# cvigilv/SimSpread.jl

Hardware: AMD Instinct MI355X
Metric: predicted edges/sec + achieved HBM GB/s, W*R SpMM (higher is better)
Workload: dtype f32

## Files before the change

simspread.jl_amd/csrc/assemble.hip:

```cpp
#include <cstdlib>
#include <cstring>
#include <hip/hip_runtime.h>
#include <rocprim/rocprim.hpp>

#include "graph.hpp"

namespace ss {

static inline int grid_for(int64_t work, int block, int cap = 256 * 16) {
  int64_t g = ceil_div(work, block);
  if (g < 1) g = 1;
  if (g > cap) g = cap;
  return (int)g;
}

__global__ void scan_tail_kernel(const int* in, int* out, int64_t n) { out[n] = out[n - 1] + in[n - 1]; }

static int exclusive_scan_int(const int* in, int* out, int64_t n) {
  hipStream_t st = ctx().stream;
  if (n == 0) {
    SS_HIP(hipMemsetAsync(out, 0, sizeof(int), st));
    return SS_OK;
  }
  size_t bytes = 0;
// ... 1124 lines not shown
    const int64_t r = i - (int64_t)c * rows;
    const int64_t o = (int64_t)off[i] * align;
    const int npad = (off[i + 1] - off[i]) * align;
    if (npad == 0) continue;
    const int lo = ptr[r], hi = ptr[r + 1];
    const int64_t k0 = (int64_t)c * SC, k1 = k0 + SC;
    int a = lo, b = hi;
    while (a < b) { const int m = (a + b) >> 1; if (idx[m] < k0) a = m + 1; else b = m; }
    const int first = a;
    b = hi;
    while (a < b) { const int m = (a + b) >> 1; if (idx[m] < k1) a = m + 1; else b = m; }
    const int n = a - first;
    if (cls_tails && n > 64) {
      const int cls = (int)(r & 3);
      int m = 0;
      for (int x0 = 0; x0 < n; x0 += 64) {
        const int x = x0 + lane;
        m += __popcll(__ballot(x < n && ((idx[first + x] - k0) & 3) == cls));
      }
      const ChunkTail tl = chunk_tail(n, m);
      int seen_c = 0, seen_o = 0;
      for (int x0 = 0; x0 < n; x0 += 64) {
        const int x = x0 + lane;
        const bool valid = x < n;
        const int col = valid ? (int)(idx[first + x] - k0) : 0;
        const T v = valid ? val[first + x] : T(0);
        const unsigned long long mc = __ballot(valid && (col & 3) == cls);
        const int rc = seen_c + __popcll(mc & below);
        const bool in_tail = valid && (col & 3) == cls && rc < tl.real;
        const unsigned long long mo = __ballot(valid && !in_tail);
        const int ro = seen_o + __popcll(mo & below);
        if (in_tail) {
          oidx[o + 64 + rc] = (unsigned short)col;
          oval[o + 64 + rc] = v;
        } else if (valid) {
          if (ro < 64) {
            hcol[wv][ro] = col;
            hval[wv][ro] = v;
          } else {
            oidx[o + 16 + ro] = (unsigned short)col;
            oval[o + 16 + ro] = v;
          }
        }
        seen_c += __popcll(mc);
        seen_o += __popcll(mo);
      }
      for (int x = tl.real + lane; x < tl.len; x += 64) {
        oidx[o + 64 + x] = (unsigned short)SC;
        oval[o + 64 + x] = T(0);
      }
      __builtin_amdgcn_wave_barrier();
      const int hc = hcol[wv][lane];
      const T hv = hval[wv][lane];
      __builtin_amdgcn_wave_barrier();
      const int pos = sched ? chunk_sched_pos(64, hc, lane) : lane;
      oidx[o + pos] = (unsigned short)hc;
      oval[o + pos] = hv;
      for (int x = tl.stored + lane; x < npad; x += 64) {
        oidx[o + x] = (unsigned short)SC;
        oval[o + x] = T(0);
      }
      continue;
    }
    if (sched && n > 32 && n <= 64) {
      const int col = lane < n ? (int)(idx[first + lane] - k0) : -1;
      const int pos = chunk_sched_pos(n, col, lane);
      if (lane < n) {
        oidx[o + pos] = (unsigned short)col;
        oval[o + pos] = val[first + lane];
      }
      for (int x = n + lane; x < npad; x += 64) {
        oidx[o + x] = (unsigned short)SC;
        oval[o + x] = T(0);
      }
      continue;
    }
    for (int x = lane; x < npad; x += 64) {
      oidx[o + x] = x < n ? (unsigned short)(idx[first + x] - k0) : (unsigned short)SC;
      oval[o + x] = x < n ? val[first + x] : T(0);
    }
  }
}

template <class T>
int chunked_build(const DevCsr<T>& in, int SC, int align, DevChunked<T>& out) {
  hipStream_t st = ctx().stream;
  if (SC < 1 || SC > 65535) return fail(SS_EINVAL, "chunk size out of range");
  if (align != 1 && align != 4 && align != 32) return fail(SS_EINVAL, "chunk alignment must be 1, 4 or 32");
  out.rows = in.rows;
  out.cols = in.cols;
  out.nnz = in.nnz;
  out.SC = SC;
  out.align = align;
  out.binary = in.binary;
  out.nchunks = (int)(in.cols > 0 ? ceil_div(in.cols, SC) : 1);
  const int64_t total = in.rows * out.nchunks;
  SS_TRY(out.off.alloc(total + 1));
  if (total == 0) {
    SS_HIP(hipMemsetAsync(out.off.p, 0, sizeof(int), st));
    SS_TRY(out.idx.alloc(64));
    SS_TRY(out.val.alloc(64));
    SS_HIP(hipMemsetAsync(out.idx.p, 0, 64 * sizeof(unsigned short), st));
    SS_HIP(hipMemsetAsync(out.val.p, 0, 64 * sizeof(T), st));
    return SS_OK;
  }
  DevBuf<int> cnt;
  SS_TRY(cnt.alloc(total));
  const int cls_tails = (align == 1 || align == 32) ? 1 : 0;
  DevBuf<int> toolong;
  if (align == 32) {
    SS_TRY(out.len.alloc(total));
    SS_TRY(toolong.alloc(1));
    SS_HIP(hipMemsetAsync(toolong.p, 0, sizeof(int), st));
  }
  hipLaunchKernelGGL(chunk_count_kernel, dim3(grid_for(total, 256)), dim3(256), 0, st, in.ptr.p, in.idx.p, in.rows, SC,
                     out.nchunks, align, cls_tails, cnt.p, align == 32 ? out.len.p : (unsigned short*)nullptr,
                     align == 32 ? toolong.p : (int*)nullptr);
  SS_LAUNCH_CHECK();
  if (align == 32) {
    int tl = 0;
    SS_TRY(read_int(toolong.p, &tl));
    out.len_ok = (tl == 0);
  }
  {
    DevBuf<int> mm;
    SS_TRY(mm.alloc(2));
    const int init[2] = {0, 0x7f7fffff};
    SS_HIP(hipMemcpyAsync(mm.p, init, sizeof(init), hipMemcpyHostToDevice, st));
    if (in.nnz > 0) {
      hipLaunchKernelGGL(abs_range_kernel<T>, dim3(grid_for(in.nnz, 256)), dim3(256), 0, st, in.val.p, in.nnz, mm.p);
      SS_LAUNCH_CHECK();
    }
    int got[2];
    SS_HIP(hipMemcpyAsync(got, mm.p, sizeof(got), hipMemcpyDeviceToHost, st));
    SS_HIP(hipStreamSynchronize(st));
    memcpy(&out.vmax, &got[0], 4);
    memcpy(&out.vmin, &got[1], 4);
    if (in.nnz == 0) out.vmax = out.vmin = 0.f;
  }
  SS_TRY(exclusive_scan_int(cnt.p, out.off.p, total));
  int units = 0;
  SS_TRY(read_int(out.off.p + total, &units));
  if (units < 0 || (int64_t)units * align >= (1LL << 31) - 64) return fail(SS_EUNSUPPORTED, "chunked operand too large");
  out.stored = (int64_t)units * align;
  SS_TRY(out.idx.alloc(out.stored + 256));
  SS_TRY(out.val.alloc(out.stored + 256));
  SS_HIP(hipMemsetAsync(out.idx.p + out.stored, 0, 256 * sizeof(unsigned short), st));
  SS_HIP(hipMemsetAsync(out.val.p + out.stored, 0, 256 * sizeof(T), st));
  const int sched = (cls_tails && !env_off("SS_CHUNK_SCHED")) ? 1 : 0;
  hipLaunchKernelGGL(chunk_fill_kernel<T>, dim3(grid_for(total * 64, 256)), dim3(256), 0, st, in.ptr.p, in.idx.p,
                     in.val.p, in.rows, SC, out.nchunks, align, sched, cls_tails, out.off.p, out.idx.p, out.val.p);
  SS_LAUNCH_CHECK();
  SS_HIP(hipStreamSynchronize(st));
  return SS_OK;
}

template <class T>
__global__ void degree_kernel(const int* __restrict__ pa, const int* __restrict__ pb, int64_t n, int* __restrict__ k,
                              T* __restrict__ inv) {
  for (int64_t i = (int64_t)blockIdx.x * blockDim.x + threadIdx.x; i < n; i += (int64_t)gridDim.x * blockDim.x) {
    int d = pa[i + 1] - pa[i];
    if (pb) d += pb[i + 1] - pb[i];
    k[i] = d;
    inv[i] = d > 0 ? T(1) / T(d) : T(0);
  }
}

template <class T>
int graph_finalize(Graph<T>& g) {
  SS_TRY(csr_transpose(g.Xs, g.XsT));
  SS_TRY(csr_transpose(g.Ys, g.YsT));
  return graph_degrees(g);
}

template <class T>
int graph_degrees(Graph<T>& g) {
  hipStream_t st = ctx().stream;
  g.coef_drop();
  SS_TRY(g.kf.alloc(g.nf));
  SS_TRY(g.ks.alloc(g.ns));
  SS_TRY(g.kt.alloc(g.nt));
  SS_TRY(g.inv_kf.alloc(g.nf));
  SS_TRY(g.inv_ks.alloc(g.ns));
  SS_TRY(g.inv_kt.alloc(g.nt));
  if (g.nf > 0) {
    hipLaunchKernelGGL(degree_kernel<T>, dim3(grid_for(g.nf, 256)), dim3(256), 0, st, g.XsT.ptr.p, (const int*)nullptr,
                       g.nf, g.kf.p, g.inv_kf.p);
    SS_LAUNCH_CHECK();
  }
  if (g.ns > 0) {
    hipLaunchKernelGGL(degree_kernel<T>, dim3(grid_for(g.ns, 256)), dim3(256), 0, st, g.Xs.ptr.p, g.Ys.ptr.p, g.ns,
                       g.ks.p, g.inv_ks.p);
    SS_LAUNCH_CHECK();
  }
  if (g.nt > 0) {
    hipLaunchKernelGGL(degree_kernel<T>, dim3(grid_for(g.nt, 256)), dim3(256), 0, st, g.YsT.ptr.p, (const int*)nullptr,
                       g.nt, g.kt.p, g.inv_kt.p);
    SS_LAUNCH_CHECK();
  }
  SS_HIP(hipStreamSynchronize(st));
  return SS_OK;
}

template <class T>
int graph_finalize_general(Graph<T>& g) {
  hipStream_t st = ctx().stream;
  const int64_t n = g.ns;
  g.coef_drop();
  SS_TRY(g.kf.alloc(n));
  SS_TRY(g.inv_kf.alloc(n));
  SS_TRY(g.ks.alloc(n));
  SS_TRY(g.inv_ks.alloc(n));
  SS_TRY(g.kt.alloc(g.nt));
  SS_TRY(g.inv_kt.alloc(g.nt));
  if (n > 0) {
    hipLaunchKernelGGL(degree_kernel<T>, dim3(grid_for(n, 256)), dim3(256), 0, st, g.XsT.ptr.p, (const int*)nullptr, n,
                       g.kf.p, g.inv_kf.p);
    SS_LAUNCH_CHECK();
    hipLaunchKernelGGL(degree_kernel<T>, dim3(grid_for(n, 256)), dim3(256), 0, st, g.XsT.ptr.p, (const int*)nullptr, n,
                       g.ks.p, g.inv_ks.p);
    SS_LAUNCH_CHECK();
  }
  if (g.nt > 0) {
    hipLaunchKernelGGL(degree_kernel<T>, dim3(grid_for(g.nt, 256)), dim3(256), 0, st, g.YsT.ptr.p, (const int*)nullptr,
                       g.nt, g.kt.p, g.inv_kt.p);
    SS_LAUNCH_CHECK();
  }
  SS_HIP(hipStreamSynchronize(st));
  return SS_OK;
}

template <class T>
int graph_finalize_general_targets(Graph<T>& g) {
  hipStream_t st = ctx().stream;
  g.coef_drop();
// ... 26 lines not shown
```

simspread.jl_amd/csrc/graph.hpp:

```cpp
#pragma once
#include "common.hpp"

#include <type_traits>

namespace ss {

template <class T>
struct DevCsr {
  int64_t rows = 0, cols = 0, nnz = 0;
  DevBuf<int> ptr;
  DevBuf<int> idx;
  DevBuf<T> val;
  bool binary = false;
};

constexpr int SELL_Q1_STEP = 8;
constexpr int SELL_LEND_R = 3;
constexpr unsigned SELL_REC_NONE = 0x00ffffffu;

template <class T>
struct DevSell {
  int64_t rows = 0, cols = 0;
  int KC = 0;
  int qt = 0;
  int nchunks = 0;
  int nslices = 0;
  int64_t nquads = 0;
  bool binary = false;
  DevBuf<int> off;
  DevBuf<unsigned short> idx;
  DevBuf<T> val;
  DevBuf<int> q1;
  DevBuf<unsigned> rec;
  bool lends = false;
  bool sorted = false;
  int64_t vrows = 0;
  DevBuf<int> vs, ve;
  DevBuf<int> vfirst;
  DevBuf<int> inv;
};

template <class T>
struct DevChunked {
  int64_t rows = 0, cols = 0, nnz = 0;
  int64_t stored = 0;
  bool binary = false;
  int SC = 0, nchunks = 0;
  int align = 1;
  DevBuf<int> off;
  DevBuf<unsigned short> idx;
  DevBuf<T> val;
  DevBuf<unsigned short> len;
  bool len_ok = false;
  float vmax = 0.f, vmin = 0.f;
};

template <class T>
struct DevCsell {
  int64_t rows = 0, cols = 0, nnz = 0;
  int KC = 0, nchunks = 0, nslices = 0;
  int QT = 0;
  bool binary = false;
  bool ok = false;
  int64_t npairs = 0;
  DevBuf<int> desc;
  DevBuf<unsigned short> np;
  DevBuf<unsigned> pidx;
  DevBuf<T> pval;
};

template <class T>
struct DenseSim {
  bool on = false;
  int64_t nq = 0, ns = 0, nf = 0;
  T alpha = T(0);
  bool weighted = true;
  DevBuf<T> Sq, Ss;
  DevBuf<T> inv_kf_m1;
  DevBuf<unsigned short> Bpl, Apl;
  int Bpl_np = 0;
  int64_t Bpl_Np = 0, Bpl_Kp = 0;
};

template <class T>
struct CoefTable {
  DevBuf<T> c;
  uint64_t epoch = 0;
  void drop() { c.release(); epoch = 0; }
};

template <class T>
struct Graph {
  int64_t nq = 0, ns = 0, nf = 0, nt = 0;
  bool general = false;
  DenseSim<T> dense;
  DevCsr<T> Xq;
  DevCsr<T> Xs;
  DevCsr<T> XsT;
  DevCsr<T> Ys;
  DevCsr<T> YsT;
  DevBuf<int> kf, ks, kt;
  DevBuf<T> inv_kf, inv_ks, inv_kt;
  DevSell<T> W;
  int W_qt = 0;
  DevChunked<T> XsTc, YsTc;
  DevChunked<T> XsTb;
  DevBuf<T> Cq;
  CoefTable<T> coef_q, coef_s, coef_y, coef_loo;
  uint64_t coef_epoch = 1;
  void coef_drop() {
    coef_q.drop(); coef_s.drop(); coef_y.drop(); coef_loo.drop();
    ++coef_epoch;
  }
  DevBuf<T> Tws;
  DevBuf<T> Sws;
};

template <class T>
struct SpMat {
  DevCsr<T> csr;
  DevSell<T> sell;
  int sell_qt = 0;
  DevChunked<T> narrow[3];
  DevChunked<T> col[3];
  DevCsell<T> csell[6];
  bool csell_tried[6] = {false, false, false, false, false, false};
  DevBuf<T> partial;
};

template <class T>
int csr_from_user(int64_t rows, int64_t cols, const int64_t* ptr, const int32_t* idx, const T* val,
                  int index_base, int mem, DevCsr<T>& out);
template <class T>
int csr_from_dense(const T* S, int64_t rows, int64_t cols, int64_t ld, bool apply_cutoff, T alpha,
                   bool weighted, int mem, DevCsr<T>& out);
template <class T>
// ... 382 lines not shown
```

simspread.jl_amd/csrc/transfer.hip:

```cpp
#include <type_traits>

#include "graph.hpp"

namespace ss {

template <class T>
struct ChunkedView {
  const int* off;
  const unsigned short* idx;
  const T* val;
  int64_t rows;
};
template <class T>
static inline ChunkedView<T> view(const DevChunked<T>& m) {
  return ChunkedView<T>{m.off.p, m.idx.p, m.val.p, m.rows};
}

template <class T>
struct TransferArgs {
  int nterms;
  CsrView<T> L[2];
  const T* inv1[2];
  const T* coef[2];
  ChunkedView<T> M[2];
  const T* inv2;
  const int* kf;
  const int* ks;
  int64_t row_begin;
  const int* row_ids;
  int64_t nj;
  int SC;
  int nchunks;
  T* out;
  int64_t ld;
  int accumulate;
  float xmax;
  int chunk_interleave;
};
template <class T>
__device__ __forceinline__ bool chunks_in_turn(const TransferArgs<T>& p) { return p.chunk_interleave != 0; }

template <class F>
static int dispatch_bool(bool b, F&& f) {
  return b ? f(std::true_type{}) : f(std::false_type{});
}
template <int... Vs, class F>
static int dispatch_int(int v, F&& f) {
  int rc = SS_OK;
  const bool hit = ((v == Vs && ((rc = f(std::integral_constant<int, Vs>{})), true)) || ...);
  return hit ? rc : fail(SS_EINVAL, "dispatch_int: no kernel for the value %d", v);
}

template <auto Kernel, class... Args>
static int launch_lds(unsigned grid, int block, size_t lds, Args... args) {
  static std::atomic<bool> attr_done{false};
  if (!attr_done) {
    SS_HIP(hipFuncSetAttribute(reinterpret_cast<const void*>(Kernel), hipFuncAttributeMaxDynamicSharedMemorySize,
                               160 * 1024));
    attr_done = true;
  }
  hipLaunchKernelGGL(Kernel, dim3(grid), dim3(block), lds, ctx().stream, args...);
  SS_LAUNCH_CHECK();
  return SS_OK;
}

constexpr int TRANSFER_THREADS = 64;

template <class T> struct BitsOf;
template <> struct BitsOf<float> {
  static __device__ __forceinline__ float bcast(float v, int src) {
    return __int_as_float(__builtin_amdgcn_readlane(__float_as_int(v), src));
  }
  static __device__ __forceinline__ float push(int to4, float v) {
    return __int_as_float(__builtin_amdgcn_ds_permute(to4, __float_as_int(v)));
  }
  static __device__ __forceinline__ float pull(int from4, float v) {
    return __int_as_float(__builtin_amdgcn_ds_bpermute(from4, __float_as_int(v)));
  }
};
template <> struct BitsOf<double> {
  static __device__ __forceinline__ double join(int lo, int hi) {
    return __longlong_as_double(((long long)hi << 32) | (unsigned int)lo);
  }
  static __device__ __forceinline__ double bcast(double v, int src) {
    const long long b = __double_as_longlong(v);
    const int lo = __builtin_amdgcn_readlane((int)(b & 0xffffffffll), src);
    const int hi = __builtin_amdgcn_readlane((int)(b >> 32), src);
    return join(lo, hi);
  }
  static __device__ __forceinline__ double push(int to4, double v) {
    const long long b = __double_as_longlong(v);
    return join(__builtin_amdgcn_ds_permute(to4, (int)(b & 0xffffffffll)), __builtin_amdgcn_ds_permute(to4, (int)(b >> 32)));
  }
  static __device__ __forceinline__ double pull(int from4, double v) {
    const long long b = __double_as_longlong(v);
    return join(__builtin_amdgcn_ds_bpermute(from4, (int)(b & 0xffffffffll)), __builtin_amdgcn_ds_bpermute(from4, (int)(b >> 32)));
  }
};
// ... 109 lines not shown
  const unsigned long long longs = __ballot(lng);
  t.nr = 0;
  if (longs == 0ull) return;
  const int cls = a_l & 3;
  int k = 0, rounds = 0, fewest = 16, spare = 0, taken = 0;
#pragma unroll
  for (int c = 0; c < 4; ++c) {
    const unsigned long long mc = __ballot(lng && cls == c);
    const int kc = (int)__builtin_amdgcn_mbcnt_hi((unsigned)(mc >> 32), __builtin_amdgcn_mbcnt_lo((unsigned)mc, 0u));
    int cc = __builtin_popcountll(mc);
    cc = cc < 16 ? cc : 16;
    k = cls == c ? kc : k;
    rounds = cc > rounds ? cc : rounds;
    if (cc < fewest) { fewest = cc; spare = 4 * cc + c; }
    taken = (lane & 3) == c ? cc : taken;
  }
  const bool placed = lng && k < 16;
  t.nr = rounds;
  t.ovf = __ballot(lng && k >= 16);
  const int to4 = (placed ? 4 * k + cls : spare) * 4;
  const bool mine = (lane >> 2) < taken;
  const int pb = __builtin_amdgcn_ds_permute(to4, b_l), pn = __builtin_amdgcn_ds_permute(to4, n_l);
  t.cb = mine ? pb : 0;
  t.cn = mine ? pn : 0;
  t.ccf = BitsOf<T>::push(to4, cf_l);
  tails_fetch(t, 0, lane, ld);
}

template <class T, bool BINM, bool FIX, int TAIL_AHEAD, class LD>
__device__ __forceinline__ void tails_finish(Tails<T, TAIL_AHEAD>& t, int b_l, int n_l, T cf_l, T* __restrict__ acc, int dummy,
                                             const unsigned short* __restrict__ midx, const T* __restrict__ mval, int lane,
                                             LD&& ld) {
  if (t.nr == 0) return;
  for (int r0 = 0; r0 < t.nr; r0 += TAIL_AHEAD) {
    if (r0 > 0) tails_fetch(t, r0, lane, ld);
#pragma unroll
    for (int i = 0; i < TAIL_AHEAD; ++i) {
      if (r0 + i >= t.nr) break;
      const int from4 = (4 * (r0 + i) + (lane >> 4)) * 4;
      const int tn = __builtin_amdgcn_ds_bpermute(from4, t.cn) - 64;
      const T tcf = BitsOf<T>::pull(from4, t.ccf);
      const bool live = (lane & 15) < tn;
      if constexpr (FIX) {
        atomicAdd(reinterpret_cast<unsigned*>(acc) + (live ? (int)t.tj[i] : dummy),
                  (unsigned)cvt_rpi(live ? (float)(tcf * t.tv[i]) : 0.f));
      } else {
        const int j = live ? (int)t.tj[i] : dummy;
        acc[j] = fma(tcf, t.tv[i], acc[j]);
      }
    }
  }
  unsigned long long m = __ballot(n_l > 80) | t.ovf;
  while (m != 0ull) {
    const int src = __builtin_ctzll(m);
    m &= m - 1ull;
    const int n = __builtin_amdgcn_readlane(n_l, src);
    const unsigned b = (unsigned)__builtin_amdgcn_readlane(b_l, src);
    const T cf = BitsOf<T>::bcast(cf_l, src);
    for (int x = (((t.ovf >> src) & 1ull) ? 64 : 80) + lane; x < n; x += 64) {
      const int j = midx[b + x];
      const T v = BINM ? T(1) : mval[b + x];
      if constexpr (FIX) atomicAdd(reinterpret_cast<unsigned*>(acc) + j, (unsigned)cvt_rpi((float)(cf * v)));
      else acc[j] = fma(cf, v, acc[j]);
    }
  }
}

struct FixedScale {
  float scale, unscale;
};
template <class F>
__device__ __forceinline__ FixedScale fixed_scale(int lb, int le, int lane, float xmax, F&& abs_coef) {
  float sabs = 0.f;
  for (int q = lb + lane; q < le; q += 64) sabs += abs_coef(q);
#pragma unroll
  for (int o = 32; o > 0; o >>= 1) sabs += __shfl_xor(sabs, o);
  int e = 0;
  (void)frexpf(sabs * xmax, &e);
  if (!(sabs * xmax > 0.f)) e = 0;
  e = e < -90 ? -90 : (e > 120 ? 120 : e);
  return FixedScale{ldexpf(1.f, 30 - e), ldexpf(1.f, e - 30)};
}

template <class T, bool LOO, int U, bool BINM, bool DUAL, bool FIX = false, bool BUF = false, bool COEF = false>
__global__ void __launch_bounds__(TRANSFER_THREADS) transfer_kernel(TransferArgs<T> p) {
  static_assert(64 % (2 * U) == 0, "U must divide 32");
  static_assert(!COEF || (!DUAL && !FIX && !BUF), "coefficient tables serve the default family only");
  extern __shared__ __align__(16) unsigned char smem_raw[];
  T* acc = reinterpret_cast<T*>(smem_raw);
  const int astride = p.SC + 64;
  constexpr int NCOPY = DUAL ? 2 : 1;
  unsigned* bits = reinterpret_cast<unsigned*>(acc + NCOPY * astride);
  const int lane = threadIdx.x;
  int c;
  int64_t r;
  if (p.nchunks > 8 && p.nchunks % 8 == 0 && !chunks_in_turn(p)) {
    const int64_t nrows = (int64_t)gridDim.x / p.nchunks, per = nrows * 8;
    const int64_t grp = blockIdx.x / per, rem = blockIdx.x - grp * per;
    r = rem >> 3;
    c = (int)(grp * 8 + (rem & 7));
  } else {
    c = blockIdx.x % p.nchunks;
    r = blockIdx.x / p.nchunks;
  }
  const int64_t gr = p.row_ids ? (int64_t)p.row_ids[p.row_begin + r] : p.row_begin + r;
  const int64_t j0 = (int64_t)c * p.SC;
  const int jn = (int)((p.nj - j0 < p.SC) ? (p.nj - j0) : p.SC);
  const int dummy = p.SC + lane;

  for (int j = lane; j < NCOPY * astride; j += 64) acc[j] = T(0);
  if (LOO)
    for (int j = lane; j < (p.SC + 31) / 32; j += 64) bits[j] = 0u;
  __syncthreads();

  float fix_unscale = 1.f;
  for (int t = 0; t < p.nterms; ++t) {
    const CsrView<T> L = p.L[t];
    const ChunkedView<T> M = p.M[t];
    const int* __restrict__ off = M.off + (int64_t)c * M.rows;
    const unsigned short* __restrict__ midx = M.idx;
    const T* __restrict__ mval = M.val;
    const int lb = L.ptr[gr], le = L.ptr[gr + 1];
    float scale = 1.f;
    if constexpr (FIX) {
      float sabs = 0.f;
      for (int q = lb + lane; q < le; q += 64) sabs += fabsf((float)(L.val[q] * p.inv1[t][L.idx[q]]));
#pragma unroll
      for (int o = 32; o > 0; o >>= 1) sabs += __shfl_xor(sabs, o);
      int e = 0;
      (void)frexpf(sabs * p.xmax, &e);
      if (!(sabs * p.xmax > 0.f)) e = 0;
      e = e < -90 ? -90 : (e > 120 ? 120 : e);
      scale = ldexpf(1.f, 30 - e);
      fix_unscale = ldexpf(1.f, e - 30);
    }
    for (int g0 = lb; g0 < le; g0 += 64) {
      const int q = g0 + lane;
      int a_l = 0, b_l = 0, n_l = 0;
      T cf_l = T(0);
      if constexpr (COEF) {
        if (q < le) {
          const int a = a_l = L.idx[q];
          cf_l = p.coef[t][q];
          const int o0 = off[a], o1 = off[a + 1];
          b_l = o0;
          n_l = cf_l != T(0) ? o1 - o0 : 0;
        }
      } else if (q < le) {
        const int a = a_l = L.idx[q];
        const T lv = L.val[q];
        if (LOO) {
          const int d = p.kf[a] - 1;
          cf_l = (a != (int)gr && d > 0) ? lv * (T(1) / T(d)) : T(0);
        } else {
          cf_l = lv * p.inv1[t][a];
          if constexpr (FIX) cf_l = (T)((float)cf_l * scale);
        }
        if (cf_l != T(0)) { b_l = off[a]; n_l = off[a + 1] - b_l; }
      }
      const int cnt = __builtin_amdgcn_readfirstlane((le - g0 < 64) ? (le - g0) : 64);
      SubRows<T, U> A, B;
      auto load = [&](SubRows<T, U>& sr, int first) __attribute__((always_inline)) {
        if constexpr (BUF) {
          const __amdgpu_buffer_rsrc_t ridx = __builtin_amdgcn_make_buffer_rsrc((void*)midx, 0, -1, 0x00020000);
          const __amdgpu_buffer_rsrc_t rval = __builtin_amdgcn_make_buffer_rsrc((void*)mval, 0, -1, 0x00020000);
          subrows_load_buf<U, BINM>(sr, first, b_l, n_l, cf_l, ridx, rval, lane);
        } else {
          subrows_load<T, U, BINM>(sr, first, b_l, n_l, cf_l, midx, mval, lane);
        }
      };
      auto tail_ld = [&](unsigned e, unsigned short& j, T& v) __attribute__((always_inline)) {
        if constexpr (BUF) {
          const __amdgpu_buffer_rsrc_t ridx = __builtin_amdgcn_make_buffer_rsrc((void*)midx, 0, -1, 0x00020000);
          const __amdgpu_buffer_rsrc_t rval = __builtin_amdgcn_make_buffer_rsrc((void*)mval, 0, -1, 0x00020000);
          j = __builtin_amdgcn_raw_buffer_load_b16(ridx, (int)(e * 2u), 0, 0);
          v = BINM ? 1.f : __builtin_bit_cast(float, __builtin_amdgcn_raw_buffer_load_b32(rval, (int)(e * 4u), 0, 0));
        } else {
          j = midx[e];
          v = BINM ? T(1) : mval[e];
        }
      };
      Tails<T, (BINM ? 4 : (DUAL || FIX || BUF) ? 2 : 3)> tails;
      tails_begin(tails, a_l, b_l, n_l, cf_l, lane, tail_ld);
      load(A, 0);
      for (int u0 = 0; u0 < cnt; u0 += 2 * U) {
        if (u0 + U < cnt) load(B, u0 + U);
        subrows_fold_any<T, U, DUAL, FIX>(A, acc, astride, dummy, lane);
        if (u0 + U < cnt) {
          if (u0 + 2 * U < cnt) load(A, u0 + 2 * U);
          subrows_fold_any<T, U, DUAL, FIX>(B, acc, astride, dummy, lane);
        }
      }
      tails_finish<T, BINM, FIX>(tails, b_l, n_l, cf_l, acc, dummy, midx, mval, lane, tail_ld);
    }
  }
  if (LOO) {
    const ChunkedView<T> M = p.M[0];
    const int* off = M.off + (int64_t)c * M.rows;
    for (int x = off[gr] + lane; x < off[gr + 1]; x += 64) {
      const int j = M.idx[x];
      if (j < p.SC) atomicOr(&bits[j >> 5], 1u << (j & 31));
    }
  }
  __syncthreads();

  T* orow = p.out + r * p.ld + j0;
  for (int j = lane; j < jn; j += 64) {
    T z;
    T sum = DUAL ? acc[j] + acc[astride + j] : acc[j];
    if constexpr (FIX) sum = (T)((float)reinterpret_cast<const int*>(acc)[j] * fix_unscale);
    if (LOO) {
      const int d = p.ks[j0 + j] - (int)((bits[j >> 5] >> (j & 31)) & 1u);
      z = (d > 0 && (j0 + j) != gr) ? sum * (T(1) / T(d)) : T(0);
    } else {
      z = sum * p.inv2[j0 + j];
      if (p.accumulate) z += orow[j];
    }
    orow[j] = z;
  }
}

constexpr int TRANSFER_U = 8;

static bool transfer_dual() { return env_int("SS_TRANSFER_DUAL", 0) != 0; }

static int transfer_u() {
  const int u = (int)env_int("SS_TRANSFER_U", TRANSFER_U);
  return (u == 4 || u == 16) ? u : 8;
}

template <class T>
__global__ void transfer_coef_kernel(const int* __restrict__ ptr, const int* __restrict__ idx, const T* __restrict__ val,
                                     const T* __restrict__ inv1, int64_t row_begin, int64_t nrows, T* __restrict__ coef) {
  const int lo = ptr[row_begin], hi = ptr[row_begin + nrows];
  for (int64_t e = (int64_t)lo + (int64_t)blockIdx.x * blockDim.x + threadIdx.x; e < hi; e += (int64_t)gridDim.x * blockDim.x)
    coef[e] = val[e] * inv1[idx[e]];
}

enum { TB_PLAIN, TB_QFLAT, TB_WIDE, TB_WIDE2 };
constexpr int WIDE_META = 64 * 12;
constexpr int WIDE_LIST = 64;
constexpr int W2_TBL = 64 * 12;
template <int KIND, class T>
struct BlockLayout {
  static constexpr bool EXACT = KIND != TB_PLAIN;
  static constexpr int shared_bytes = KIND == TB_WIDE ? 64 : 0;
  __host__ __device__ static int64_t offs_bytes(int64_t mrows) { return (((mrows + 1) * 4 + 15) / 16) * 16; }
  __host__ __device__ static int64_t lens_bytes(int64_t mrows) { return EXACT ? ((mrows * 2 + 15) / 16) * 16 : 0; }
  __host__ __device__ static int acc_elems(int SC) { return SC + 64; }
  __host__ __device__ static int acc_bytes(int SC) {
    return KIND == TB_WIDE || KIND == TB_WIDE2 ? (((SC + 4) * 4 + 15) / 16) * 16 : acc_elems(SC) * (int)sizeof(T);
  }
  __host__ __device__ static int per_wave(int SC) {
    return acc_bytes(SC) + (KIND == TB_WIDE ? WIDE_META + WIDE_LIST : KIND == TB_WIDE2 ? 2 * W2_TBL + 4 * 64 : 0);
  }
  __device__ static unsigned char* wave_base(unsigned char* smem, int offs_b, int lens_b, int wave, int SC) {
    return smem + offs_b + lens_b + shared_bytes + (size_t)wave * (size_t)per_wave(SC);
  }
};

struct BlockWave {
  int lane, c, jn, lb, le;
  int64_t r, gr, j0;
};

template <bool EXACT, class T, class A>
__device__ __forceinline__ bool block_prologue(BlockWave& w, const TransferArgs<T>& p, int64_t nrows, int wave, int* offs,
                                               unsigned short* lens, const unsigned short* glen, A* acc, int nacc) {
  const int nw = blockDim.x >> 6;
  w.lane = threadIdx.x & 63;
  w.c = blockIdx.x % p.nchunks;
  w.r = (int64_t)(blockIdx.x / p.nchunks) * nw + wave;
  const ChunkedView<T> M = p.M[0];
  {
    const int* __restrict__ off = M.off + (int64_t)w.c * M.rows;
    for (int64_t i = threadIdx.x; i <= M.rows; i += blockDim.x) offs[i] = off[i];
    if constexpr (EXACT) {
      const unsigned short* __restrict__ gl = glen + (int64_t)w.c * M.rows;
      for (int64_t i = threadIdx.x; i < M.rows; i += blockDim.x) lens[i] = gl[i];
    }
  }
  for (int j = w.lane; j < nacc; j += 64) acc[j] = A(0);
// ... 533 lines not shown
  SS_LAUNCH_CHECK();
  constexpr bool CANFIX = std::is_same<T, float>::value;
  const bool fx = CANFIX && fixed;
  if (fx) path_add("fixed_point");
  const bool binm = Mt.binary;
  if constexpr (CANFIX) {
    const int wide2 = (int)env_int("SS_TRANSFER_WIDE2", 0), wide = (int)env_int("SS_TRANSFER_WIDE", 0),
              qflat = (int)env_int("SS_TRANSFER_QFLAT", 0);
    if ((wide2 > 0 || wide > 0 || qflat > 0) && fixed && Mt.align == 32 && Mt.len_ok) {
      if (wide2 > 0) {
        if (const int n = transfer_block_waves<TB_WIDE2, T>(Mt.rows, Mt.SC)) {
          path_add("wide2");
          return dispatch_bool(binm, [&](auto B) {
            return launch_block_kernel<TB_WIDE2, transfer_wide2_kernel<decltype(B)::value>>(p, Mt, coef, nrows, n, xmax);
          });
        }
      } else if (wide > 0) {
        if (const int n = transfer_block_waves<TB_WIDE, T>(Mt.rows, Mt.SC)) {
          path_add("wide");
          return dispatch_int<2, 4>(wide == 2 ? 2 : 4, [&](auto D) {
            return dispatch_bool(binm, [&](auto B) {
              return launch_block_kernel<TB_WIDE, transfer_wide_kernel<decltype(D)::value, decltype(B)::value>>(
                  p, Mt, coef, nrows, n, xmax);
            });
          });
        }
      } else if (const int n = transfer_block_waves<TB_QFLAT, T>(Mt.rows, Mt.SC)) {
        path_add("qflat");
        return dispatch_bool(binm, [&](auto B) {
          return launch_block_kernel<TB_QFLAT, transfer_qflat_kernel<float, 4, decltype(B)::value>>(p, Mt, coef, nrows, n, xmax);
        });
      }
    }
  }
  return dispatch_int<4, 8>(transfer_u() == 4 ? 4 : 8, [&](auto U) {
    return dispatch_bool(binm, [&](auto B) {
      return dispatch_bool(fx, [&](auto F) {
        constexpr bool FIX = CANFIX && decltype(F)::value;
        return launch_block_kernel<TB_PLAIN, transfer_block_kernel<T, decltype(U)::value, decltype(B)::value, FIX>>(
            p, Mt, coef, nrows, nw, xmax);
      });
    });
  });
}

template <class T, bool LOO>
__global__ void __launch_bounds__(256) transfer_coef_rows_kernel(CsrView<T> L, const T* __restrict__ inv1,
                                                                 const int* __restrict__ kf, int64_t nrows,
                                                                 T* __restrict__ coef) {
  for (int64_t r = blockIdx.x; r < nrows; r += gridDim.x) {
    const int lb = L.ptr[r], le = L.ptr[r + 1];
    for (int q = lb + (int)threadIdx.x; q < le; q += 256) {
      const int a = L.idx[q];
      const T lv = L.val[q];
      if (LOO) {
        const int d = kf[a] - 1;
        coef[q] = (a != (int)r && d > 0) ? lv * (T(1) / T(d)) : T(0);
      } else {
        coef[q] = lv * inv1[a];
      }
    }
  }
}

template <class T>
int transfer_coef_build(const DevCsr<T>& L, const T* inv1, const int* kf_loo, T* coef) {
  if (L.rows <= 0 || L.nnz <= 0) return SS_OK;
  const unsigned grid = (unsigned)(L.rows < 65536 ? L.rows : 65536);
  if (kf_loo)
    hipLaunchKernelGGL((transfer_coef_rows_kernel<T, true>), dim3(grid), dim3(256), 0, ctx().stream, view(L), inv1, kf_loo,
                       L.rows, coef);
  else
    hipLaunchKernelGGL((transfer_coef_rows_kernel<T, false>), dim3(grid), dim3(256), 0, ctx().stream, view(L), inv1, kf_loo,
                       L.rows, coef);
  SS_LAUNCH_CHECK();
  return SS_OK;
}

static int transfer_coef_mode() {
  const int m = (int)env_int("SS_TRANSFER_COEF", 1);
  return m == 0 ? 0 : (m == 2 ? 2 : 1);
}

template <class T, bool LOO>
static int launch_transfer_variant(const TransferArgs<T>& p, unsigned grid, size_t lds, bool binm, bool dual) {
  auto launch = [&](auto kernel) {
    hipLaunchKernelGGL(kernel, dim3(grid), dim3(TRANSFER_THREADS), lds, ctx().stream, p);
    SS_LAUNCH_CHECK();
    return (int)SS_OK;
  };
  const int u = transfer_u();
  bool coef = !dual && (u == 4 || u == 8) && transfer_coef_mode() != 0 && p.row_ids == nullptr;
  if constexpr (std::is_same<T, float>::value && !LOO)
    coef = coef && env_int("SS_TRANSFER_LD", 0) != 1 && env_int("SS_TRANSFER_FIX1", 0) != 1;
  for (int t = 0; t < p.nterms; ++t) coef = coef && p.coef[t] != nullptr;
  if (coef) {
    if (transfer_coef_mode() == 2) path_add("coef_table");
    return dispatch_int<4, 8>(u, [&](auto U) {
      return dispatch_bool(binm, [&](auto B) {
        return launch(transfer_kernel<T, LOO, decltype(U)::value, decltype(B)::value, false, false, false, true>);
      });
    });
  }
  if constexpr (std::is_same<T, float>::value && !LOO) {
    const bool buf = !dual && env_int("SS_TRANSFER_LD", 0) == 1;
    const bool fix = !dual && env_int("SS_TRANSFER_FIX1", 0) == 1 && p.nterms == 1 && !p.accumulate;
    if (buf) path_add("buffer_loads");
    if (fix) path_add("fixed_point");
    if (buf || fix)
      return dispatch_int<4, 8>(u == 4 ? 4 : 8, [&](auto U) {
        return dispatch_bool(binm, [&](auto B) {
          return dispatch_bool(fix, [&](auto F) {
            return dispatch_bool(buf, [&](auto BF) {
              return launch(transfer_kernel<T, LOO, decltype(U)::value, decltype(B)::value, false, decltype(F)::value,
                                            decltype(BF)::value>);
            });
          });
        });
      });
  }
  return dispatch_int<4, 8, 16>(u, [&](auto U) {
    return dispatch_bool(binm, [&](auto B) {
      return dispatch_bool(dual, [&](auto D) {
        return launch(transfer_kernel<T, LOO, decltype(U)::value, decltype(B)::value, decltype(D)::value>);
      });
    });
  });
}

template <class T>
int launch_transfer(int nterms, const DevCsr<T>* L[2], const T* inv1[2], const DevChunked<T>* Mt[2],
                    const T* inv2, int64_t row_begin, int64_t nrows, int64_t nj, T* out, int64_t ld,
                    const int* row_ids, bool accumulate, const T* const* coef) {
  if (nrows <= 0 || nj <= 0) return SS_OK;
  TransferArgs<T> p{};
  p.nterms = nterms;
  for (int t = 0; t < nterms; ++t) {
    p.L[t] = view(*L[t]);
    p.M[t] = view(*Mt[t]);
    p.inv1[t] = inv1[t];
    p.coef[t] = coef ? coef[t] : nullptr;
    if (Mt[t]->SC != Mt[0]->SC || Mt[t]->nchunks != Mt[0]->nchunks)
      return fail(SS_EINVAL, "transfer operands were cut with different chunk sizes");
  }
  p.inv2 = inv2;
  p.row_begin = row_begin;
  p.row_ids = row_ids;
  p.nj = nj;
  p.SC = Mt[0]->SC;
  p.nchunks = Mt[0]->nchunks;
  p.out = out;
  p.ld = ld;
  p.accumulate = accumulate ? 1 : 0;
  p.xmax = 1.0f;
  p.chunk_interleave = env_off("SS_TRANSFER_ORDER") ? 1 : 0;
  bool binm = true;
  for (int t = 0; t < nterms; ++t) binm = binm && Mt[t]->binary;
  const int64_t grid = nrows * p.nchunks;
  if (grid >= (1LL << 31)) return fail(SS_EUNSUPPORTED, "transfer grid too large; lower SS_TRANSFER_BYTES");
  const bool dual = transfer_dual();
  path_add("transfer");
  const size_t lds = (size_t)(p.SC + 64) * sizeof(T) * (dual ? 2 : 1);
  return launch_transfer_variant<T, false>(p, (unsigned)grid, lds, binm, dual);
}

template <class T>
int launch_transfer_loo(const DevCsr<T>& X, const DevChunked<T>& XT, const int* kf, const int* ks,
                        int64_t i_begin, int64_t nrows, T* out, int64_t ld, const T* coef) {
  if (nrows <= 0) return SS_OK;
  TransferArgs<T> p{};
  p.nterms = 1;
  p.L[0] = view(X);
  p.M[0] = view(XT);
  p.kf = kf;
  p.ks = ks;
  p.coef[0] = coef;
  p.row_begin = i_begin;
  p.nj = X.rows;
  p.SC = XT.SC;
  p.nchunks = XT.nchunks;
  p.out = out;
  p.ld = ld;
  p.chunk_interleave = env_off("SS_TRANSFER_ORDER") ? 1 : 0;
  const int64_t grid = nrows * p.nchunks;
  if (grid >= (1LL << 31)) return fail(SS_EUNSUPPORTED, "transfer grid too large; lower SS_TRANSFER_BYTES");
  const bool dual = transfer_dual();
  path_add("transfer_loo");
  const size_t lds = (size_t)(p.SC + 64) * sizeof(T) * (dual ? 2 : 1) + (size_t)((p.SC + 31) / 32) * 4;
  return launch_transfer_variant<T, true>(p, (unsigned)grid, lds, XT.binary, dual);
}

#define SS_INSTANTIATE(T)                                                                                   \
  template int launch_transfer<T>(int, const DevCsr<T>*[2], const T*[2], const DevChunked<T>*[2], const T*, \
                                  int64_t, int64_t, int64_t, T*, int64_t, const int*, bool, const T* const*);     \
  template int transfer_coef_build<T>(const DevCsr<T>&, const T*, const int*, T*);                          \
  template int launch_transfer_block<T>(const DevCsr<T>&, const T*, const DevChunked<T>&, const T*, int64_t, int64_t, \
                                        int64_t, T*, int64_t, T*, float, bool);                               \
  template bool transfer_block_fits<T>(int64_t, int);                                                        \
  template int launch_transfer_loo<T>(const DevCsr<T>&, const DevChunked<T>&, const int*, const int*,       \
                                      int64_t, int64_t, T*, int64_t, const T*);
SS_INSTANTIATE(float)
SS_INSTANTIATE(double)

}
```

Before: 53.63 billion.

## Compress chunked row offsets to 16-bit residuals against a linear predictor

Adds a build step that stores each chunk's row offsets as 16-bit residuals from a linear fit (slope S, bias), with a per-chunk descriptor and a fallback flag when the residual range exceeds 16 bits. The transfer kernel gains an OFF16 variant that reads both bounds with one 32-bit load and reconstructs them arithmetically. This halves the offset array footprint and gather traffic for the M operand's subrow bounds. In exchange it adds extra multiply/shift work per gather, extra build kernels and a host sync read, and doubles the kernel instantiations.

Result: no change. 53.42 billion (-0.4%).

```diff
diff --git a/simspread.jl_amd/csrc/assemble.hip b/simspread.jl_amd/csrc/assemble.hip
--- a/simspread.jl_amd/csrc/assemble.hip
+++ b/simspread.jl_amd/csrc/assemble.hip
@@ -1230,9 +1230,93 @@
   }
 }
 
+__global__ void __launch_bounds__(256) chunk_off16_describe_kernel(const int* __restrict__ off, int64_t rows,
+                                                                   int* __restrict__ desc, int* __restrict__ bad) {
+  __shared__ int smin[256], smax[256];
+  const int* __restrict__ o = off + (int64_t)blockIdx.x * rows;
+  const int base = o[0];
+  const unsigned long long span = (unsigned long long)(o[rows] - base);
+  const unsigned long long S64 = (span << 8) / (unsigned long long)rows;
+  const bool fits = S64 * (unsigned long long)rows < (1ull << 32);
+  const unsigned S = (unsigned)S64;
+  int mn = 0x7fffffff, mx = -0x7fffffff - 1;
+  if (fits)
+    for (int64_t a = threadIdx.x; a <= rows; a += 256) {
+      const int res = o[a] - base - (int)(((unsigned)a * S) >> 8);
+      mn = res < mn ? res : mn;
+      mx = res > mx ? res : mx;
+    }
+  smin[threadIdx.x] = mn;
+  smax[threadIdx.x] = mx;
+  __syncthreads();
+  for (int s = 128; s > 0; s >>= 1) {
+    if ((int)threadIdx.x < s) {
+      smin[threadIdx.x] = min(smin[threadIdx.x], smin[threadIdx.x + s]);
+      smax[threadIdx.x] = max(smax[threadIdx.x], smax[threadIdx.x + s]);
+    }
+    __syncthreads();
+  }
+  if (threadIdx.x == 0) {
+    const long long range = (long long)smax[0] - (long long)smin[0];
+    if (!fits || range > 65534) {
+      *bad = 1;
+      desc[2 * blockIdx.x] = 0;
+      desc[2 * blockIdx.x + 1] = 0;
+    } else {
+      const int bias = 32768 - (smin[0] + (int)(range >> 1));
+      desc[2 * blockIdx.x] = (int)S;
+      desc[2 * blockIdx.x + 1] = base - bias;
+    }
+  }
+}
+
+__global__ void chunk_off16_fill_kernel(const int* __restrict__ off, int64_t rows, int nchunks, int64_t stride,
+                                        const int* __restrict__ desc, unsigned short* __restrict__ off16) {
+  const int64_t total = (int64_t)nchunks * stride;
+  for (int64_t i = (int64_t)blockIdx.x * blockDim.x + threadIdx.x; i < total; i += (int64_t)gridDim.x * blockDim.x) {
+    const int c = (int)(i / stride);
+    const int64_t a = i - (int64_t)c * stride;
+    int v = 0;
+    if (a <= rows) v = off[(int64_t)c * rows + a] - (int)(((unsigned)a * (unsigned)desc[2 * c]) >> 8) - desc[2 * c + 1];
+    off16[i] = (unsigned short)v;
+  }
+}
+
+template <class T>
+static int chunked_off16(DevChunked<T>& out) {
+  hipStream_t st = ctx().stream;
+  out.off16_ok = out.off16_fallback = false;
+  if (out.rows <= 0 || out.nchunks <= 0) return SS_OK;
+  out.off16_stride = (out.rows + 2) & ~(int64_t)1;
+  SS_TRY(out.off16.alloc((size_t)(out.nchunks * out.off16_stride)));
+  SS_TRY(out.off16_desc.alloc((size_t)out.nchunks * 2));
+  DevBuf<int> bad;
+  SS_TRY(bad.alloc(1));
+  SS_HIP(hipMemsetAsync(bad.p, 0, sizeof(int), st));
+  hipLaunchKernelGGL(chunk_off16_describe_kernel, dim3(out.nchunks), dim3(256), 0, st, (const int*)out.off.p, out.rows,
+                     out.off16_desc.p, bad.p);
+  SS_LAUNCH_CHECK();
+  hipLaunchKernelGGL(chunk_off16_fill_kernel, dim3(grid_for(out.nchunks * out.off16_stride, 256)), dim3(256), 0, st,
+                     (const int*)out.off.p, out.rows, out.nchunks, out.off16_stride, (const int*)out.off16_desc.p,
+                     out.off16.p);
+  SS_LAUNCH_CHECK();
+  int b = 0;
+  SS_TRY(read_int(bad.p, &b));
+  out.off16_ok = (b == 0);
+  out.off16_fallback = (b != 0);
+  if (b != 0) {
+    out.off16.release();
+    out.off16_desc.release();
+  }
+  return SS_OK;
+}
+
 template <class T>
 int chunked_build(const DevCsr<T>& in, int SC, int align, DevChunked<T>& out) {
   hipStream_t st = ctx().stream;
+  out.off16_ok = out.off16_fallback = false;
+  out.off16.release();
+  out.off16_desc.release();
   if (SC < 1 || SC > 65535) return fail(SS_EINVAL, "chunk size out of range");
   if (align != 1 && align != 4 && align != 32) return fail(SS_EINVAL, "chunk alignment must be 1, 4 or 32");
   out.rows = in.rows;
@@ -1299,6 +1383,7 @@
   hipLaunchKernelGGL(chunk_fill_kernel<T>, dim3(grid_for(total * 64, 256)), dim3(256), 0, st, in.ptr.p, in.idx.p,
                      in.val.p, in.rows, SC, out.nchunks, align, sched, cls_tails, out.off.p, out.idx.p, out.val.p);
   SS_LAUNCH_CHECK();
+  if (align == 1 && !env_off("SS_CHUNK_OFF16")) SS_TRY(chunked_off16(out));
   SS_HIP(hipStreamSynchronize(st));
   return SS_OK;
 }
diff --git a/simspread.jl_amd/csrc/graph.hpp b/simspread.jl_amd/csrc/graph.hpp
--- a/simspread.jl_amd/csrc/graph.hpp
+++ b/simspread.jl_amd/csrc/graph.hpp
@@ -52,6 +52,11 @@
   DevBuf<T> val;
   DevBuf<unsigned short> len;
   bool len_ok = false;
+  DevBuf<unsigned short> off16;
+  DevBuf<int> off16_desc;
+  int64_t off16_stride = 0;
+  bool off16_ok = false;
+  bool off16_fallback = false;
   float vmax = 0.f, vmin = 0.f;
 };
 
diff --git a/simspread.jl_amd/csrc/transfer.hip b/simspread.jl_amd/csrc/transfer.hip
--- a/simspread.jl_amd/csrc/transfer.hip
+++ b/simspread.jl_amd/csrc/transfer.hip
@@ -10,10 +10,48 @@
   const unsigned short* idx;
   const T* val;
   int64_t rows;
+  const unsigned short* off16;
+  const int* off16_desc;
+  int64_t off16_stride;
 };
 template <class T>
 static inline ChunkedView<T> view(const DevChunked<T>& m) {
-  return ChunkedView<T>{m.off.p, m.idx.p, m.val.p, m.rows};
+  return ChunkedView<T>{m.off.p, m.idx.p, m.val.p, m.rows, m.off16_ok ? m.off16.p : nullptr, m.off16_desc.p, m.off16_stride};
+}
+
+template <bool OFF16>
+struct ChunkBounds {
+  const int* off;
+  const unsigned short* off16;
+  unsigned S;
+  int add;
+};
+template <bool OFF16, class T>
+__device__ __forceinline__ ChunkBounds<OFF16> chunk_bounds(const ChunkedView<T>& M, int c) {
+  ChunkBounds<OFF16> cb{};
+  if constexpr (OFF16) {
+    cb.off16 = M.off16 + (int64_t)c * M.off16_stride;
+    cb.S = (unsigned)M.off16_desc[2 * c];
+    cb.add = M.off16_desc[2 * c + 1];
+  } else {
+    cb.off = M.off + (int64_t)c * M.rows;
+  }
+  return cb;
+}
+template <bool OFF16>
+__device__ __forceinline__ void subrow_bounds(const ChunkBounds<OFF16>& cb, int a, int& b, int& n) {
+  if constexpr (OFF16) {
+    unsigned w;
+    __builtin_memcpy(&w, cb.off16 + a, 4);
+    const int o0 = (int)(((unsigned)a * cb.S) >> 8) + (int)(w & 0xffffu);
+    const int o1 = (int)(((unsigned)(a + 1) * cb.S) >> 8) + (int)(w >> 16);
+    b = o0 + cb.add;
+    n = o1 - o0;
+  } else {
+    const int o0 = cb.off[a], o1 = cb.off[a + 1];
+    b = o0;
+    n = o1 - o0;
+  }
 }
 
 template <class T>
@@ -289,10 +327,12 @@
   return FixedScale{ldexpf(1.f, 30 - e), ldexpf(1.f, e - 30)};
 }
 
-template <class T, bool LOO, int U, bool BINM, bool DUAL, bool FIX = false, bool BUF = false, bool COEF = false>
+template <class T, bool LOO, int U, bool BINM, bool DUAL, bool FIX = false, bool BUF = false, bool COEF = false,
+          bool OFF16 = false>
 __global__ void __launch_bounds__(TRANSFER_THREADS) transfer_kernel(TransferArgs<T> p) {
   static_assert(64 % (2 * U) == 0, "U must divide 32");
   static_assert(!COEF || (!DUAL && !FIX && !BUF), "coefficient tables serve the default family only");
+  static_assert(!OFF16 || (!DUAL && !FIX && !BUF && U <= 8), "16-bit bounds serve the default family only");
   extern __shared__ __align__(16) unsigned char smem_raw[];
   T* acc = reinterpret_cast<T*>(smem_raw);
   const int astride = p.SC + 64;
@@ -324,7 +364,7 @@
   for (int t = 0; t < p.nterms; ++t) {
     const CsrView<T> L = p.L[t];
     const ChunkedView<T> M = p.M[t];
-    const int* __restrict__ off = M.off + (int64_t)c * M.rows;
+    const ChunkBounds<OFF16> cb = chunk_bounds<OFF16>(M, c);
     const unsigned short* __restrict__ midx = M.idx;
     const T* __restrict__ mval = M.val;
     const int lb = L.ptr[gr], le = L.ptr[gr + 1];
@@ -349,9 +389,9 @@
         if (q < le) {
           const int a = a_l = L.idx[q];
           cf_l = p.coef[t][q];
-          const int o0 = off[a], o1 = off[a + 1];
-          b_l = o0;
-          n_l = cf_l != T(0) ? o1 - o0 : 0;
+          int n;
+          subrow_bounds(cb, a, b_l, n);
+          n_l = cf_l != T(0) ? n : 0;
         }
       } else if (q < le) {
         const int a = a_l = L.idx[q];
@@ -363,7 +403,7 @@
           cf_l = lv * p.inv1[t][a];
           if constexpr (FIX) cf_l = (T)((float)cf_l * scale);
         }
-        if (cf_l != T(0)) { b_l = off[a]; n_l = off[a + 1] - b_l; }
+        if (cf_l != T(0)) subrow_bounds(cb, a, b_l, n_l);
       }
       const int cnt = __builtin_amdgcn_readfirstlane((le - g0 < 64) ? (le - g0) : 64);
       SubRows<T, U> A, B;
@@ -403,8 +443,9 @@
   }
   if (LOO) {
     const ChunkedView<T> M = p.M[0];
-    const int* off = M.off + (int64_t)c * M.rows;
-    for (int x = off[gr] + lane; x < off[gr + 1]; x += 64) {
+    int xb, xn;
+    subrow_bounds(chunk_bounds<OFF16>(M, c), (int)gr, xb, xn);
+    for (int x = xb + lane; x < xb + xn; x += 64) {
       const int j = M.idx[x];
       if (j < p.SC) atomicOr(&bits[j >> 5], 1u << (j & 31));
     }
@@ -1104,6 +1145,8 @@
   return m == 0 ? 0 : (m == 2 ? 2 : 1);
 }
 
+static bool bounds16_tagged() { return env_int("SS_CHUNK_OFF16", 1) == 2; }
+
 template <class T, bool LOO>
 static int launch_transfer_variant(const TransferArgs<T>& p, unsigned grid, size_t lds, bool binm, bool dual) {
   auto launch = [&](auto kernel) {
@@ -1116,14 +1159,28 @@
   if constexpr (std::is_same<T, float>::value && !LOO)
     coef = coef && env_int("SS_TRANSFER_LD", 0) != 1 && env_int("SS_TRANSFER_FIX1", 0) != 1;
   for (int t = 0; t < p.nterms; ++t) coef = coef && p.coef[t] != nullptr;
+  bool off16 = !dual && (u == 4 || u == 8);
+  if constexpr (std::is_same<T, float>::value && !LOO)
+    off16 = off16 && env_int("SS_TRANSFER_LD", 0) != 1 && env_int("SS_TRANSFER_FIX1", 0) != 1;
+  for (int t = 0; t < p.nterms; ++t) off16 = off16 && p.M[t].off16 != nullptr;
+  if (off16 && bounds16_tagged()) path_add("bounds16");
   if (coef) {
     if (transfer_coef_mode() == 2) path_add("coef_table");
     return dispatch_int<4, 8>(u, [&](auto U) {
       return dispatch_bool(binm, [&](auto B) {
-        return launch(transfer_kernel<T, LOO, decltype(U)::value, decltype(B)::value, false, false, false, true>);
+        return dispatch_bool(off16, [&](auto O) {
+          return launch(transfer_kernel<T, LOO, decltype(U)::value, decltype(B)::value, false, false, false, true,
+                                        decltype(O)::value>);
+        });
       });
     });
   }
+  if (off16)
+    return dispatch_int<4, 8>(u, [&](auto U) {
+      return dispatch_bool(binm, [&](auto B) {
+        return launch(transfer_kernel<T, LOO, decltype(U)::value, decltype(B)::value, false, false, false, false, true>);
+      });
+    });
   if constexpr (std::is_same<T, float>::value && !LOO) {
     const bool buf = !dual && env_int("SS_TRANSFER_LD", 0) == 1;
     const bool fix = !dual && env_int("SS_TRANSFER_FIX1", 0) == 1 && p.nterms == 1 && !p.accumulate;
@@ -1182,6 +1239,8 @@
   if (grid >= (1LL << 31)) return fail(SS_EUNSUPPORTED, "transfer grid too large; lower SS_TRANSFER_BYTES");
   const bool dual = transfer_dual();
   path_add("transfer");
+  for (int t = 0; t < nterms; ++t)
+    if (Mt[t]->off16_fallback && bounds16_tagged()) { path_add("bounds32_fallback"); break; }
   const size_t lds = (size_t)(p.SC + 64) * sizeof(T) * (dual ? 2 : 1);
   return launch_transfer_variant<T, false>(p, (unsigned)grid, lds, binm, dual);
 }
@@ -1208,6 +1267,7 @@
   if (grid >= (1LL << 31)) return fail(SS_EUNSUPPORTED, "transfer grid too large; lower SS_TRANSFER_BYTES");
   const bool dual = transfer_dual();
   path_add("transfer_loo");
+  if (XT.off16_fallback && bounds16_tagged()) path_add("bounds32_fallback");
   const size_t lds = (size_t)(p.SC + 64) * sizeof(T) * (dual ? 2 : 1) + (size_t)((p.SC + 31) / 32) * 4;
   return launch_transfer_variant<T, true>(p, (unsigned)grid, lds, XT.binary, dual);
 }
```
